# stojicnnnn/3DVision

Hardware: AMD Instinct MI355X
Metric: RANSAC hyps/s + ICP iters/s @ 200k-pt clouds (higher is better)
Workload: dtype f32

## Files before the change

3dvision_amd/__init__.py:

```python
import ctypes as C
import os
import sys
import threading
from dataclasses import dataclass, field
from typing import Optional

import numpy as np

_HERE = os.path.dirname(os.path.abspath(__file__))
STUDY_BUILD = os.environ.get("TDV_LIB_VARIANT") == "study"
LIB_PATH = os.path.join(_HERE, "lib3dvision_hip_study.so" if STUDY_BUILD else "lib3dvision_hip.so")

TDV_MASK_THRESHOLD10 = 0
TDV_MASK_NONZERO = 1
TDV_MASK_LABEL_BASE = 256
TDV_VOXEL_ORDER_FIRST = 0
TDV_VOXEL_ORDER_REFERENCE = 1
TIMER_ICP_NN, TIMER_RANSAC_SCORE, TIMER_FEATURE_MATCH, TIMER_KNN, TIMER_RADIUS, TIMER_DEPTH, TIMER_VOXEL, TIMER_FM_INDEX = range(8)
DEPTH_BATCH_MASK_PASSES = 1

ABI_SYMBOLS = [
    "tdv_device_count", "tdv_ctx_create", "tdv_ctx_set_stream", "tdv_ctx_set_icp_search", "tdv_ctx_set_icp_accumulation", "tdv_ctx_last_icp_search", "tdv_ctx_last_batch_lanes", "tdv_ctx_last_voxel_grouping", "tdv_ctx_last_voxel_batch_redone", "tdv_ctx_last_feature_match_path", "tdv_ctx_workspace_bytes", "tdv_ctx_workspace_fill", "tdv_ctx_set_ransac_score", "tdv_ctx_last_ransac_rescore", "tdv_ctx_last_ransac_scored", "tdv_ctx_last_ransac_bound", "tdv_ctx_get_stream", "tdv_ctx_synchronize",
    "tdv_ctx_destroy", "tdv_status_string", "tdv_last_error", "tdv_version", "tdv_timing_enable", "tdv_timing_read",
    "tdv_depth_preprocess", "tdv_deproject", "tdv_depth_to_cloud", "tdv_voxel_downsample", "tdv_estimate_normals",
    "tdv_compute_fpfh", "tdv_feature_match", "tdv_ransac", "tdv_icp", "tdv_icp_correspondences",
    "tdv_icp_dev", "tdv_ransac_dev", "tdv_feature_match_dev", "tdv_estimate_normals_dev", "tdv_compute_fpfh_dev", "tdv_normals_fpfh_dev", "tdv_radix_sort_pairs_dev",
    "tdv_depth_to_cloud_dev", "tdv_voxel_downsample_dev", "tdv_sample_triples", "tdv_sample_triples_batch", "tdv_pose_compose",
    "tdv_register_batch_dev", "tdv_prepare_model_dev", "tdv_bilateral_filter", "tdv_filter_duplicates", "tdv_ransac_score_unit", "tdv_ransac_score_unit_block", "tdv_ransac_score_unit_chunks", "tdv_ransac_batch_size", "tdv_voxel_rules", "tdv_load_ply_ascii", "tdv_load_mask_png", "tdv_load_masks_from_dir",
    "tdv_depth_to_cloud_batch_dev", "tdv_broadcast_model", "tdv_gather_results", "tdv_mask_resize_nearest", "tdv_mask_resize_nearest_dev", "tdv_voxel_downsample_batch_dev", "tdv_voxel_downsample_batch_pinhole_dev",
    "tdv_icp_batch_dev", "tdv_refine_batch_dev", "tdv_ctx_set_icp_loss", "tdv_ctx_get_icp_loss",
    "tdv_gicp", "tdv_gicp_dev", "tdv_gicp_batch_dev",
    "tdv_color_gradients", "tdv_color_gradients_dev", "tdv_colored_icp", "tdv_colored_icp_dev", "tdv_colored_icp_batch_dev",
    "tdv_fgr_default_params", "tdv_fgr", "tdv_fgr_dev", "tdv_fgr_correspondences",
    "tdv_plane_default_params", "tdv_segment_planes", "tdv_segment_planes_dev",
    "tdv_cluster_default_params", "tdv_cluster_dbscan", "tdv_cluster_dbscan_dev",
    "tdv_remove_statistical_outlier", "tdv_remove_statistical_outlier_dev", "tdv_remove_radius_outlier", "tdv_remove_radius_outlier_dev",
    "tdv_iss_default_params", "tdv_iss_keypoints", "tdv_iss_keypoints_dev",
    "tdv_ppf_default_params", "tdv_ppf_model_bytes", "tdv_ppf_model_dev", "tdv_ppf_match_dev", "tdv_ppf_match",
    "tdv_ppf_match_batch_dev",
    "tdv_farthest_point_down_sample", "tdv_farthest_point_down_sample_dev", "tdv_farthest_point_down_sample_batch_dev",
    "tdv_ctx_set_fps_path", "tdv_ctx_last_fps_path", "tdv_ctx_set_icp_launches", "tdv_ctx_last_icp_launches",
    "tdv_ctx_set_icp_probe_cache", "tdv_ctx_last_icp_probe_misses",
    "tdv_verify_default_params", "tdv_verify_poses", "tdv_verify_poses_dev", "tdv_render_depth", "tdv_render_depth_dev",
    "tdv_mesh_verify_default_params", "tdv_verify_poses_mesh", "tdv_verify_poses_mesh_dev", "tdv_render_depth_mesh", "tdv_render_depth_mesh_dev",
    "tdv_mesh_sample_default_params", "tdv_mesh_sample_points", "tdv_mesh_sample_points_dev",
# ... 507 lines not shown
        _check(self._h, lib().tdv_ctx_set_icp_search(self._h, self.ICP_SEARCH[mode]), "tdv_ctx_set_icp_search")
        self.icp_search_name = mode

    def set_icp_accumulation(self, mode):
        _check(self._h, lib().tdv_ctx_set_icp_accumulation(self._h, {"tree": 0, "reference": 1}[mode]), "tdv_ctx_set_icp_accumulation")

    ICP_LOSS = {"l2": 0, "huber": 1, "tukey": 2, "cauchy": 3}

    def set_icp_loss(self, kind, scale=None):
        if kind not in self.ICP_LOSS:
            raise ValueError("unknown ICP loss %r (one of %s)" % (kind, ", ".join(self.ICP_LOSS)))
        if kind != "l2" and scale is None:
            raise ValueError("the %s loss needs a scale" % kind)
        _check(self._h, lib().tdv_ctx_set_icp_loss(self._h, self.ICP_LOSS[kind], C.c_float(0.0 if scale is None else float(scale))),
               "tdv_ctx_set_icp_loss")

    def icp_loss(self):
        k = C.c_int(); sc = C.c_float()
        _check(self._h, lib().tdv_ctx_get_icp_loss(self._h, C.byref(k), C.byref(sc)), "tdv_ctx_get_icp_loss")
        return {v: n for n, v in self.ICP_LOSS.items()}[k.value], float(sc.value)

    def set_ransac_score(self, mode):
        _check(self._h, lib().tdv_ctx_set_ransac_score(self._h, {"fast": 0, "exact": 1, "matrix": 2}[mode]), "tdv_ctx_set_ransac_score")

    def last_ransac_rescore(self):
        return float(lib().tdv_ctx_last_ransac_rescore(self._h))

    def last_ransac_scored(self):
        return float(lib().tdv_ctx_last_ransac_scored(self._h))

    def last_ransac_bound(self):
        out = (C.c_longlong * 4)()
        lib().tdv_ctx_last_ransac_bound(self._h, out)
        return tuple(int(v) for v in out)

    def last_feature_match_path(self):
        return {0: "none", 1: "scan", 2: "leaf_major", 3: "walk"}[int(lib().tdv_ctx_last_feature_match_path(self._h))]

    def last_voxel_grouping(self):
        return {0: "none", 1: "table", 2: "pixels"}[int(lib().tdv_ctx_last_voxel_grouping(self._h))]

    def last_voxel_batch_redone(self):
        return int(lib().tdv_ctx_last_voxel_batch_redone(self._h))

    def last_batch_lanes(self):
        return int(lib().tdv_ctx_last_batch_lanes(self._h))
# ... 1247 lines not shown
```

3dvision_amd/csrc/batch.hip:

```cpp
#include "tdv_internal.hpp"
#include <algorithm>
#include <functional>
#include <thread>
#include <cstdio>
#include <cstdlib>
#include <cstring>
#include <vector>

namespace tdv {

__global__ void k_globalise(const int* __restrict__ local, const int* __restrict__ voff, int n_inst, int total, int* __restrict__ out) {
    const int P = blockIdx.x * blockDim.x + threadIdx.x;
    if (P >= total) return;
    int a = 0, z = n_inst;
    while (z - a > 1) { const int m = (a + z) >> 1; if (voff[m] <= P) a = m; else z = m; }
    out[P] = local[P] + voff[a];
}

__global__ void k_gather_i32(const int* __restrict__ in, const int* __restrict__ idx, int n, int* __restrict__ out) {
    const int p = blockIdx.x * blockDim.x + threadIdx.x;
    if (p < n) out[p] = in[idx[p]];
}

namespace {
// ... 223 lines not shown
    const bool small_instances = off[n_instances] / std::max(n_instances, 1) < 8192;
    const int lanes_default = std::min(small_instances ? 12 : 3, hw_threads);
    const int want = std::max(1, std::min(std::min(lanes_env > 0 ? lanes_env : lanes_default, 16), n_instances));
    std::vector<tdv_ctx*> lane_ctx{ctx};
    for (tdv_ctx* c = ctx; (int)lane_ctx.size() < want; c = c->helper) {
        if (!c->helper && tdv_ctx_create(ctx->device, &c->helper) != TDV_OK) { c->helper = nullptr; break; }
        lane_ctx.push_back(c->helper);
    }
    const int L = (int)lane_ctx.size();
    ctx->last_batch_lanes = L;
    auto for_all_instances = [&](const std::function<int(tdv_ctx*, int)>& fn) -> int {
        if (L == 1) {
            int st = TDV_OK;
            for (int b = 0; b < n_instances && st == TDV_OK; ++b) st = fn(ctx, b);
            if (hipStreamSynchronize(ctx->stream) != hipSuccess && st == TDV_OK) st = TDV_ERR_LAUNCH;
            return st;
        }
        TDV_HIP(ctx, hipStreamSynchronize(ctx->stream));
        std::vector<int> status((size_t)L, TDV_OK);
        std::vector<std::thread> workers;
        for (int l = 1; l < L; ++l) {
            tdv_ctx* h = lane_ctx[l];
            h->timing = ctx->timing; h->icp_search = ctx->icp_search; h->icp_accumulate = ctx->icp_accumulate;
            h->icp_loss = ctx->icp_loss; h->icp_loss_scale = ctx->icp_loss_scale; h->ransac_score_mode = ctx->ransac_score_mode; h->err[0] = 0;
            workers.emplace_back([&, h, l]() {
                try {
                    if (hipSetDevice(h->device) != hipSuccess) { status[l] = TDV_ERR_NO_DEVICE; return; }
                    status[l] = ws_reset(h);
                    for (int b = l; b < n_instances && status[l] == TDV_OK; b += L) status[l] = fn(h, b);
                    if (hipStreamSynchronize(h->stream) != hipSuccess && status[l] == TDV_OK) status[l] = TDV_ERR_LAUNCH;
                } catch (...) {
                    std::snprintf(h->err, sizeof(h->err), "exception in a helper lane");
                    status[l] = TDV_ERR_INTERNAL;
                }
            });
        }
        try {
            for (int b = 0; b < n_instances && status[0] == TDV_OK; b += L) status[0] = fn(ctx, b);
        } catch (...) {
            std::snprintf(ctx->err, sizeof(ctx->err), "exception in the batch lane");
            status[0] = TDV_ERR_INTERNAL;
        }
        for (auto& w : workers) w.join();
        if (hipStreamSynchronize(ctx->stream) != hipSuccess && status[0] == TDV_OK) status[0] = TDV_ERR_LAUNCH;
        if (status[0] != TDV_OK) return status[0];
        for (int l = 1; l < L; ++l)
            if (status[l] != TDV_OK) { std::snprintf(ctx->err, sizeof(ctx->err), "batch lane %d: %s", l + 1, lane_ctx[l]->err); return status[l]; }
// ... 247 lines not shown
```

3dvision_amd/csrc/ctx.hip:

```cpp
#include "tdv_internal.hpp"
#include <cmath>
#include <cfloat>
#include <algorithm>
#include <cstring>
#include <vector>

namespace tdv {

int ws_reset(tdv_ctx* ctx) {
    if (ctx->blocks.size() > 1) {
        size_t total = 0;
        TDV_HIP(ctx, hipStreamSynchronize(ctx->stream));
        for (auto& b : ctx->blocks) { total += b.cap; (void)hipFree(b.p); }
        ctx->blocks.clear();
        total = align_up(total + total / 4, (size_t)1 << 20);
        char* p = nullptr;
        TDV_HIP(ctx, hipMalloc((void**)&p, total));
        ctx->blocks.push_back({p, total});
    }
    ctx->cur_block = 0; ctx->cur_off = 0; ctx->used_total = 0;
    return TDV_OK;
}

int ws_alloc_bytes(tdv_ctx* ctx, size_t bytes, void** out) {
// ... 274 lines not shown
    if (!ctx || loss < TDV_ICP_LOSS_L2 || loss > TDV_ICP_LOSS_CAUCHY) return TDV_ERR_BAD_ARG;
    if (loss != TDV_ICP_LOSS_L2 && !(std::isfinite(scale) && scale > 0.f)) return TDV_ERR_BAD_ARG;
    ctx->icp_loss = loss;
    ctx->icp_loss_scale = loss == TDV_ICP_LOSS_L2 ? 0.f : scale;
    return TDV_OK;
}

int tdv_ctx_get_icp_loss(tdv_ctx* ctx, int* loss, float* scale) {
    if (!ctx) return TDV_ERR_BAD_ARG;
    if (loss) *loss = ctx->icp_loss;
    if (scale) *scale = ctx->icp_loss_scale;
    return TDV_OK;
}

int tdv_ctx_set_icp_search(tdv_ctx* ctx, int mode) {
    if (!ctx || mode < TDV_ICP_SEARCH_AUTO || mode > TDV_ICP_SEARCH_GRID) return TDV_ERR_BAD_ARG;
    ctx->icp_search = mode;
    return TDV_OK;
}

int tdv_ctx_set_ransac_score(tdv_ctx* ctx, int mode) {
    if (!ctx || (mode != TDV_RANSAC_SCORE_FAST && mode != TDV_RANSAC_SCORE_EXACT && !(tdv::kStudyBuild && mode == TDV_RANSAC_SCORE_MATRIX))) return TDV_ERR_BAD_ARG;
    ctx->ransac_score_mode = mode;
    return TDV_OK;
}

int tdv_ctx_set_fps_path(tdv_ctx* ctx, int mode) {
    if (!ctx || mode < TDV_FPS_AUTO || mode > TDV_FPS_GRID) return TDV_ERR_BAD_ARG;
    ctx->fps_path = mode;
    return TDV_OK;
}
int tdv_ctx_last_fps_path(tdv_ctx* ctx) { return ctx ? ctx->last_fps_path : 0; }

double tdv_ctx_last_ransac_rescore(tdv_ctx* ctx) { return ctx ? ctx->last_ransac_rescore : -1.0; }

double tdv_ctx_last_ransac_scored(tdv_ctx* ctx) { return ctx ? ctx->last_ransac_scored : 1.0; }
void tdv_ctx_last_ransac_bound(tdv_ctx* ctx, long long out[4]) { if (out) for (int e = 0; e < 4; ++e) out[e] = ctx ? ctx->last_ransac_bound[e] : 0; }

int tdv_ctx_last_icp_search(tdv_ctx* ctx) { return ctx ? ctx->last_icp_search : 0; }
int tdv_ctx_last_feature_match_path(tdv_ctx* ctx) { return ctx ? ctx->last_fm_path : 0; }
int tdv_ctx_last_voxel_grouping(tdv_ctx* ctx) { return ctx ? ctx->last_voxel_grouping : 0; }
int tdv_ctx_last_voxel_batch_redone(tdv_ctx* ctx) { return ctx ? ctx->last_voxel_batch_redone : TDV_ERR_BAD_ARG; }
int tdv_ctx_last_batch_lanes(tdv_ctx* ctx) { return ctx ? ctx->last_batch_lanes : 0; }
unsigned long long tdv_ctx_workspace_bytes(tdv_ctx* ctx) {
    unsigned long long total = 0;
    for (tdv_ctx* c = ctx; c; c = c->helper)
// ... 122 lines not shown
```

3dvision_amd/csrc/ransac.hip:

```cpp
#include "tdv_internal.hpp"
#include "host_wait.hpp"
#include "device_linalg.hpp"
#include "ransac_cut.hpp"
#include <cfloat>
#include <climits>
#include <cmath>
#include <cstddef>
#include <cstring>
#include <algorithm>
#include <type_traits>
#include <vector>

namespace tdv {

constexpr float kUnitRoundoff = 5.9604644775390625e-08f;
constexpr float kBandUnit = 16.f * kUnitRoundoff;
constexpr float kBandUnitMatrix = 24.f * kUnitRoundoff;

template <class I>
__device__ __forceinline__ float pair_record(const float* __restrict__ src, const float* __restrict__ tgt, const int* __restrict__ corr, I i, int nt,
                                             int* __restrict__ bad, float4& a, float4& b) {
    int c = corr[i];
    if ((unsigned)c >= (unsigned)nt) { *bad = 1; c = 0; }
    a = make_float4(src[3 * i], src[3 * i + 1], src[3 * i + 2], tgt[3 * c]);
// ... 817 lines not shown
            const int leaf = i / RL_LEAF;
            rl_leaf_store(leaves + (size_t)(leaf >> 1) * 32 + (leaf & 1), min(RL_LEAF, ns - i), bad, lo, hi);
        }
    }
    __syncthreads();
    const int k = threadIdx.x;
    const int i0 = blockIdx.x * 256 + k * RL_COARSE;
    if (k >= 256 / RL_COARSE || i0 >= ns) return;
    float clo[6], chi[6];
    bool cbad = false;
#pragma unroll
    for (int c = 0; c < 6; ++c) { clo[c] = INFINITY; chi[c] = -INFINITY; }
#pragma unroll
    for (int j = 0; j < PER; ++j) {
#pragma unroll
        for (int c = 0; c < 6; ++c) { clo[c] = fminf(clo[c], s_lo[k * PER + j][c]); chi[c] = fmaxf(chi[c], s_hi[k * PER + j][c]); }
        cbad |= s_bad[k * PER + j] != 0;
    }
    const int leaf = i0 / RL_COARSE;
    rl_leaf_store(coarse + (size_t)(leaf >> 1) * 32 + (leaf & 1), min(RL_COARSE, ns - i0), cbad, clo, chi);
}
constexpr int RB_SPLIT = 16;
enum { RB_ONE = 0, RB_COARSE = 1 };
__device__ __forceinline__ int rb_walk(const float* r, const float* __restrict__ leaves, int k0, int k1, float tb, int best, bool done) {
    int ub = 0;
    v2f rr[12], ar[9];
#pragma unroll
    for (int e = 0; e < 12; ++e) rr[e] = (v2f){r[e], r[e]};
#pragma unroll
    for (int e = 0; e < 9; ++e) ar[e] = (v2f){fabsf(r[e]), fabsf(r[e])};
    for (int k = k0; k < k1; ++k) {
        if (((k - k0) & 7) == 0 && !__any(!done)) break;
        const float* __restrict__ g = leaves + (size_t)k * 32;
        float v[32];
#pragma unroll
        for (int e = 0; e < 32; ++e) v[e] = g[e];
        const v2f pcx = {v[0], v[1]}, pcy = {v[2], v[3]}, pcz = {v[4], v[5]};
        const v2f pex = {v[8], v[9]}, pey = {v[10], v[11]}, pez = {v[12], v[13]};
        v2f g2 = {0.f, 0.f};
#pragma unroll
        for (int c = 0; c < 3; ++c) {
            const v2f xc = fma2(rr[c], pcx, fma2(rr[3 + c], pcy, fma2(rr[6 + c], pcz, rr[9 + c])));
            const v2f xe = fma2(ar[c], pex, fma2(ar[3 + c], pey, ar[6 + c] * pez));
            const v2f qlo = {v[16 + 2 * c], v[17 + 2 * c]}, qhi = {v[24 + 2 * c], v[25 + 2 * c]};
            const v2f lo_gap = (xc - xe) - qhi, hi_gap = qlo - (xc + xe);
            const v2f gp = {fmaxf(fmaxf(lo_gap.x, hi_gap.x), 0.f), fmaxf(fmaxf(lo_gap.y, hi_gap.y), 0.f)};
            g2 = fma2(gp, gp, g2);
        }
        const int n2 = (!(g2.x > tb) ? (int)v[6] : 0) + (!(g2.y > tb) ? (int)v[7] : 0);
        if (!done) { ub += n2; done = ub > best; }
    }
    return ub;
}
struct RbHyp { float r[12]; float tb, E; bool bounded; };
__device__ __forceinline__ float rb_band(const float* r, const unsigned* __restrict__ pmax, float sqrt_tau, float band_u) {
    return (band_u * ransac_band_reach(r, __uint_as_float(*pmax)) + band_u * sqrt_tau) * 1.0001f;
// ... 100 lines not shown
    const bool valid = h < count && triples.valid(h);
    const RbHyp o = rb_load(hyp, h_pad, h, valid, pmax, sqrt_tau, band_u, MODE == RB_COARSE ? 5.f : 3.f);
    const int best = state[0];
    const bool walk = rb_gate(best, ns);
    int fl = 0;
    if (wave == 0 && valid) fl = lj.flags[h];
    const int per = (n_lpairs + RB_SPLIT - 1) / RB_SPLIT, k0 = __builtin_amdgcn_readfirstlane(wave) * per, k1 = min(n_lpairs, k0 + per);
    const int ub = rb_walk(o.r, leaves, k0, k1, o.tb, best, !valid || !o.bounded || !walk);
    __syncthreads();
    if (ub) atomicAdd(&s_ub[lane], ub);
    __syncthreads();
    if (wave != 0) return;
    const int total = s_ub[lane];
    const bool gated = valid && (!o.bounded || !walk);
    const bool close = (fl & RB_CLOSE) != 0;
    const bool undecided = MODE == RB_COARSE && valid && !gated && !close && total > best;
    const bool is_live = gated || close || (MODE == RB_ONE && valid && total > best);
    const bool near = is_live && lj.near && (fl & RB_NEAR);
    const unsigned long long mc = __ballot(close);
    if (mc && lane == 0) atomicAdd(lj.n_close, __popcll(mc));
    const int slot = rb_append3(is_live && !near, near, undecided, lane, h, live, n_live, lj.near, lj.n_near, und, n_und);
    if (MODE == RB_COARSE && undecided) acc[slot] = 0;
}
constexpr int RB_FINE_Y = 4;
__global__ __launch_bounds__(64 * RB_SPLIT)
void k_ransac_bound_fine(const float* __restrict__ hyp, int h_pad, const float* __restrict__ leaves, int n_lpairs,
                         const unsigned* __restrict__ pmax, float sqrt_tau, float band_u, const int* __restrict__ state,
                         int* __restrict__ live, int* __restrict__ n_live, const int* __restrict__ und, const int* __restrict__ n_und,
                         int* __restrict__ acc, int* __restrict__ ticket, const ListJob lj) {
    const int lane = threadIdx.x & 63, wave = threadIdx.x >> 6;
    const int n = *n_und, best = state[0];
    const int per_y = (n_lpairs + (int)gridDim.y - 1) / (int)gridDim.y, y0 = blockIdx.y * per_y, y1 = min(n_lpairs, y0 + per_y);
    const int per = (y1 - y0 + RB_SPLIT - 1) / RB_SPLIT;
    const int k0 = min(y1, y0 + __builtin_amdgcn_readfirstlane(wave) * per), k1 = min(y1, k0 + per);
    __shared__ int s_ub[64];
    const int xb = blockIdx.x;
    if (xb * 64 >= n) return;
    const int slot = xb * 64 + lane;
    const int h = slot < n ? und[slot] : -1;
    if (wave == 0) s_ub[lane] = 0;
    const RbHyp o = rb_load(hyp, h_pad, h, h >= 0, pmax, sqrt_tau, band_u, 3.f);
    const int ub = rb_walk(o.r, leaves, k0, k1, o.tb, best, h < 0);
    __syncthreads();
    if (ub) atomicAdd(&s_ub[lane], ub);
    __syncthreads();
    if (wave != 0) return;
    const int part = s_ub[lane];
    if (h >= 0 && part) atomicAdd(&acc[slot], part);
    __threadfence();
    int arrived = 0;
    if (lane == 0) arrived = atomicAdd(&ticket[xb], 1);
    if (__shfl(arrived, 0, 64) != (int)gridDim.y - 1) return;
    const int total = h >= 0 ? atomicAdd(&acc[slot], 0) : 0;
    const bool is_live = h >= 0 && total > best;
    const bool near = is_live && lj.near && (lj.flags[h] & RB_NEAR);
    rb_append3(is_live && !near, near, false, lane, h, live, n_live, lj.near, lj.n_near, nullptr, nullptr);
}

#ifdef TDV_STUDY
#include "ransac_study.hpp"
#endif

__global__ __launch_bounds__(256)
void k_ransac_rmse_partial(const float* __restrict__ pq, int ns, const float* __restrict__ hyp12, float tau,
                           double* __restrict__ slabs) {
    const int i = blockIdx.x * 256 + threadIdx.x;
    double e = 0.0, n = 0.0;
    if (i < ns) {
        const float* g = pq + (size_t)i * 8;
        float px = g[0], py = g[1], pz = g[2];
        float x = (hyp12[0] * px + (hyp12[3] * py + hyp12[6] * pz)) + hyp12[9];
        float y = (hyp12[1] * px + (hyp12[4] * py + hyp12[7] * pz)) + hyp12[10];
        float z = (hyp12[2] * px + (hyp12[5] * py + hyp12[8] * pz)) + hyp12[11];
        float dx = x - g[3], dy = y - g[4], dz = z - g[5];
        float d2 = dx * dx + (dy * dy + dz * dz);
        if (d2 < tau) { float err = sqrtf(d2); e = (double)(err * err); n = 1.0; }
    }
    __shared__ double red[2][4];
#pragma unroll
// ... 46 lines not shown

struct RansacBlock {
    int bad;
    unsigned pmax;
    unsigned long long rescored, scored;
    long long bound[4];
    int state[2];
    int plan[2][8];
    float best12[12];
    double out2[2];
    int sel[4];
    int rec[2][8];
    RansacFar far;
};
constexpr size_t kRansacReadBack = offsetof(RansacBlock, sel);
static_assert(std::is_trivially_copyable<RansacBlock>::value, "memset, copied back");
static_assert(offsetof(RansacBlock, rescored) % 8 == 0 && offsetof(RansacBlock, scored) == offsetof(RansacBlock, rescored) + 8, "the kernels index the two as one u64[2]");
static_assert(offsetof(RansacBlock, out2) % 8 == 0 && offsetof(RansacBlock, out2) + sizeof(double[2]) == kRansacReadBack, "the part read back is a prefix that ends with out2");
struct RansacLive { int n_live[2], n_und[2], n_near[2], n_close[2]; };
static_assert(offsetof(RansacLive, n_und) == offsetof(RansacLive, n_live) + 2 * sizeof(int) && offsetof(RansacLive, n_near) == offsetof(RansacLive, n_live) + 4 * sizeof(int) &&
              offsetof(RansacLive, n_close) == offsetof(RansacLive, n_live) + 6 * sizeof(int), "ransac_plan's n_live[2], n_live[4], n_live[6]");

struct RansacKnobs { bool score_fast, score_mfma, bailout, bound, one_level, leaf_classes, merge, record_copy, upload_inline, order, far, end_event, timer_events; int drop_permille, a_permille, u_cut_permille, fine_y, grown; float far_radius, live_radius; };
static RansacKnobs ransac_knobs(const tdv_ctx* ctx, bool traced, int max_iterations) {
    RansacKnobs k;
    static const bool score_exact_env = getenv("TDV_RANSAC_SCORE") && !strcmp(getenv("TDV_RANSAC_SCORE"), "exact");
    k.score_fast = !score_exact_env && ctx->ransac_score_mode != TDV_RANSAC_SCORE_EXACT;
    const bool score_mfma_env = study_env("TDV_RANSAC_SCORE") && !strcmp(study_env("TDV_RANSAC_SCORE"), "mfma");
    k.score_mfma = kStudyBuild && k.score_fast && (score_mfma_env || ctx->ransac_score_mode == TDV_RANSAC_SCORE_MATRIX);
    static const bool bailout_env_off = getenv("TDV_RANSAC_BAILOUT") && atoi(getenv("TDV_RANSAC_BAILOUT")) == 0;
    k.bailout = k.score_fast && !k.score_mfma && !traced && !bailout_env_off && max_iterations > 16384;
    k.merge = study_env("TDV_RANSAC_MERGE") && atoi(study_env("TDV_RANSAC_MERGE")) == 1;
    const bool bound_env_off = getenv("TDV_RANSAC_BOUND") && atoi(getenv("TDV_RANSAC_BOUND")) == 0;
    k.bound = k.bailout && !k.merge && !bound_env_off;
    const char* const order_env = getenv("TDV_RANSAC_ORDER");
    k.order = k.bailout && !k.merge && !(order_env && atoi(order_env) == 0);
    k.far = k.order && k.bound && !(order_env && atoi(order_env) == 1);
    k.far_radius = study_env("TDV_RANSAC_FAR_RADIUS") ? (float)atof(study_env("TDV_RANSAC_FAR_RADIUS")) : 4.f;
    k.a_permille = study_env("TDV_RANSAC_FAR_A_PERMILLE") ? atoi(study_env("TDV_RANSAC_FAR_A_PERMILLE")) : 110;
    k.u_cut_permille = study_env("TDV_RANSAC_FAR_UCUT_PERMILLE") ? atoi(study_env("TDV_RANSAC_FAR_UCUT_PERMILLE")) : 22;
    k.live_radius = study_env("TDV_RANSAC_LIVE_RADIUS") ? (float)atof(study_env("TDV_RANSAC_LIVE_RADIUS")) : 20.f;
    k.fine_y = study_env("TDV_RANSAC_FINE_Y") ? std::min(std::max(atoi(study_env("TDV_RANSAC_FINE_Y")), 1), 64) : RB_FINE_Y;
    k.grown = study_env("TDV_RANSAC_GROWN") ? (int)align_up((size_t)std::min(std::max(atoi(study_env("TDV_RANSAC_GROWN")), kRansacBatch), 4 * kRansacBatch), RS_HYP_PER_BLOCK) : kRansacGrown;
    k.leaf_classes = study_env("TDV_RANSAC_LEAF_CLASSES") && atoi(study_env("TDV_RANSAC_LEAF_CLASSES")) == 1;
    k.one_level = study_env("TDV_RANSAC_BOUND_LEVELS") && atoi(study_env("TDV_RANSAC_BOUND_LEVELS")) == 1;
    k.record_copy = study_env("TDV_RANSAC_RECORD") && !strcmp(study_env("TDV_RANSAC_RECORD"), "copy");
    k.end_event = traced || k.record_copy || (study_env("TDV_RANSAC_END") && !strcmp(study_env("TDV_RANSAC_END"), "event"));
    k.timer_events = study_env("TDV_RANSAC_TIMER") && !strcmp(study_env("TDV_RANSAC_TIMER"), "events");
    k.upload_inline = study_env("TDV_RANSAC_UPLOAD") && !strcmp(study_env("TDV_RANSAC_UPLOAD"), "inline");
    k.drop_permille = study_env("TDV_RANSAC_DROP_PERMILLE") ? atoi(study_env("TDV_RANSAC_DROP_PERMILLE")) : 50;
    return k;
}

struct RansacBuf {
    float* hyp; int* counts; void* tri; int* list;
    int *live, *und, *acc, *ticket;
    int *near, *list2, *ubf;
    int* flags;
    int* units;
    int *plan, *rec, *n_live, *n_und, *n_near;
    void* h_tri; int* h_cnt; volatile int* h_rec;
    hipEvent_t ev;
    int seq;
};
struct RansacBatch { int q, cnt, it0; bool bounded; };
struct RangeCut { int per, ranges; };
static RangeCut range_cut(int hb, int n_pchunks) {
    const int per = (n_pchunks + point_ranges(hb, n_pchunks) - 1) / point_ranges(hb, n_pchunks);
    return RangeCut{per, (n_pchunks + per - 1) / per};
}
static int hyp_blocks(int cnt) { return (int)(align_up((size_t)cnt, RS_HYP_PER_BLOCK) / RS_HYP_PER_BLOCK); }
static int score_grid(int hb, int ps) { return 8 * ((hb + 8 / RS_XCD_R - 1) / (8 / RS_XCD_R)) * ((ps + RS_XCD_R - 1) / RS_XCD_R); }
static int unit_grid(int cus) { return std::max(8, (2 * cus + 7) / 8 * 8); }

struct RansacRun {
    tdv_ctx* ctx; hipStream_t s; RansacKnobs k;
    int ns, nt, max_iterations; float confidence; int* trace;
    float tau, sqrt_tau, band_u;
    int ns_pad, n_pchunks, batch, cap, h_pad, packed, rblocks, n_lpairs = 0, n_cpairs = 0, cus = 0;
    size_t tri_bytes;
    float *pq = nullptr, *pq2 = nullptr, *pq3 = nullptr, *leaves = nullptr, *cleaves = nullptr; double* slabs = nullptr;
    RansacBlock *d = nullptr, *h = nullptr; RansacLive* lv = nullptr;
    unsigned long long* leaf_keys = nullptr; unsigned* leaf_vals = nullptr; bool leaves_built = false;
    unsigned long long* ord_mask = nullptr; int* ord_cnt = nullptr; bool ordered = false;
    unsigned* enc = nullptr;
    RansacBuf buf[2] = {};
    unsigned long long *stamps = nullptr, *h_stamps = nullptr; int n_stamps = 0, stamps_used = 0;
    RansacBatch pending = {}; bool has_pending = false;
    double wave_chunks = 0.0;
    float best_fitness = 0.f; int best_iter = -1, best_inliers = 0, done_iters = 0; bool stop = false;

    TriView tri(const RansacBuf& B) const { return TriView{B.tri, packed}; }
    int setup(const float* d_src, const float* d_tgt, const int* d_corr) {
        ns_pad = (int)align_up((size_t)ns, (size_t)RS_PCH * 64);
        TDV_TRY(ws_alloc(ctx, (size_t)ns_pad * 8, &pq)); TDV_TRY(ws_alloc(ctx, 1, &d));
        TDV_HIP(ctx, hipMemsetAsync(d, 0, sizeof(RansacBlock), s));
// ... 109 lines not shown
        if (k.score_mfma) wave_chunks += mfma_score(s, B.hyp, h_pad, pq3, ns, b.cnt, tau, B.counts, &d->rescored);
        else
#endif
        if (k.score_fast) {
            const ScoreJob ja{B.hyp, B.counts, nullptr, nullptr, hb, range_cut(hb, n_pchunks).ranges, nullptr, nullptr, nullptr};
            const int gA = score_grid(hb, ja.ps);
            launch_score(gA, ja, ja, gA);
            wave_chunks += (double)hb * (RS_BLOCK / 64) * (double)n_pchunks;
        } else {
            const RangeCut c = range_cut(h_pad / RS_HYP_PER_BLOCK, n_pchunks);
            k_ransac_score<<<dim3(hb, c.ranges), RS_BLOCK, 0, s>>>(B.hyp, h_pad, pq2, n_pchunks, c.per, tau, B.counts);
        }
        return TDV_OK;
    }
    void bound(const RansacBatch& b) {
        const RansacBuf& B = buf[b.q]; const int bgrid = (b.cnt + 63) / 64;
        const ListJob lj{B.flags, k.far ? B.near : nullptr, B.n_near, B.n_live + 6};
        if (k.one_level)
            k_ransac_bound<RB_ONE><<<bgrid, 64 * RB_SPLIT, 0, s>>>(B.hyp, h_pad, tri(B), b.cnt, leaves, n_lpairs, &d->pmax, sqrt_tau, band_u,
                                                                   d->state, ns, B.live, B.n_live, nullptr, nullptr, nullptr, nullptr, lj);
        else {
            k_ransac_bound<RB_COARSE><<<bgrid, 64 * RB_SPLIT, 0, s>>>(B.hyp, h_pad, tri(B), b.cnt, cleaves, n_cpairs, &d->pmax, sqrt_tau, band_u,
                                                                      d->state, ns, B.live, B.n_live, B.und, B.n_und, B.acc, B.ticket, lj);
            k_ransac_bound_fine<<<dim3(bgrid, k.fine_y), 64 * RB_SPLIT, 0, s>>>(B.hyp, h_pad, leaves, n_lpairs, &d->pmax, sqrt_tau, band_u,
                                                                                  d->state, B.live, B.n_live, B.und, B.n_und, B.acc, B.ticket, lj);
        }
    }
    void point_order() {
        RansacFar* const far = k.far ? &d->far : nullptr;
        k_order_flags<<<order_blocks(), RO_BLOCK, 0, s>>>(pq, ns, d->state, d->best12, tau, ord_mask, ord_cnt, far, std::max(tau, k.far_radius * k.far_radius * tau));
        k_order_scatter<<<order_blocks(), RO_BLOCK, 0, s>>>(pq, ns, ord_mask, ord_cnt, pq2, far);
        ordered = true;
    }
    ScoreJob job_a(const RansacBatch& b) const { return ScoreJob{buf[b.q].hyp, buf[b.q].counts, buf[b.q].plan, nullptr, hyp_blocks(b.cnt), range_cut(hyp_blocks(b.cnt), n_pchunks).ranges, nullptr, nullptr, nullptr}; }
    void phase1(const RansacBatch& b) {
        const RansacBuf& B = buf[b.q];
        const int hbw = slots(b.cnt) / RS_BLOCK;
        const ScoreJob ja = job_a(b), jl{B.hyp, B.counts, B.plan, B.live, hbw, 0, B.n_live, B.units, nullptr};
        const ScoreJob jn = k.far ? ScoreJob{B.hyp, B.counts, B.plan, B.near, hbw, 0, B.n_near, B.units + 16 * hbw, &d->far.c_far} : jl;
        const int g1 = score_grid(ja.hb, ja.ps);
        ScopedTimer tm(ctx, score_slot());
        if (b.bounded) launch_score(unit_grid(cus), jn, jl, 0);
        else launch_score(g1, ja, ja, g1);
    }
    int select(const RansacBatch& b) {
        const RansacBuf& B = buf[b.q];
        if (b.bounded) k_ransac_select_live<<<1, 1024, 0, s>>>(B.live, B.n_live, k.far ? B.near : nullptr, B.n_near, B.ubf, B.counts, ns, confidence, d->state, B.plan, B.list, B.list2);
        else {
// ... 146 lines not shown
        pose_to_T16(h->best12, out->T);
        out->fitness = best_fitness; out->inliers = best_inliers; out->best_iteration = best_iter;
        out->rmse = best_inliers > 0 ? std::sqrt((float)h->out2[0] / (float)best_inliers) : 999.0f;
        if ((int)(h->out2[1] + 0.5) != best_inliers) {
            snprintf(ctx->err, sizeof(ctx->err), "ransac: rmse pass counted %d inliers, scoring pass %d", (int)(h->out2[1] + 0.5), best_inliers);
            return TDV_ERR_INTERNAL;
        }
        return TDV_OK;
    }
};

int ransac_run_dev(tdv_ctx* ctx, const float* d_src, int ns, const float* d_tgt, int nt, const float* d_fs, const float* d_ft, const int* d_corr_in,
                   float voxel, int max_iterations, float confidence, uint32_t seed, tdv_ransac_result* out, int* trace_inliers) {
    if (!ctx || !out || ns < 0 || nt < 0 || max_iterations < 0) return TDV_ERR_BAD_ARG;
    if (ns > 0 && (!d_src || !d_tgt)) return TDV_ERR_BAD_ARG;
    if (!d_corr_in && ns > 0 && nt > 0 && (!d_fs || !d_ft)) return TDV_ERR_BAD_ARG;
    TDV_HIP(ctx, hipSetDevice(ctx->device));
    result_defaults(out);
    if (ns == 0 || nt == 0 || max_iterations == 0) return TDV_OK;
    int* d_match = nullptr;
    if (!d_corr_in) { TDV_TRY(ws_alloc(ctx, (size_t)ns, &d_match)); TDV_TRY(feature_match_dev(ctx, d_fs, ns, d_ft, nt, d_match)); }
    const int* d_corr = d_corr_in ? d_corr_in : d_match;
    RansacRun r;
    r.ctx = ctx; r.s = ctx->stream; r.k = ransac_knobs(ctx, trace_inliers != nullptr, max_iterations);
    r.ns = ns; r.nt = nt; r.max_iterations = max_iterations; r.confidence = confidence; r.trace = trace_inliers;
    r.tau = tau_lt(voxel * 1.5f);
    r.sqrt_tau = std::nextafter((float)std::sqrt((double)r.tau), INFINITY);
    r.band_u = r.k.score_mfma ? kBandUnitMatrix : kBandUnit;
    TDV_TRY(r.setup(d_src, d_tgt, d_corr));
    const int status = r.loop(seed);
    (void)hipStreamSynchronize(r.s);
    ctx->last_ransac_rescore = -1.0; ctx->last_ransac_scored = 1.0;
    for (long long& v : ctx->last_ransac_bound) v = 0;
    r.release_events();
    return status != TDV_OK ? status : r.result(out);
}


struct RbResult { float T[12]; int best_iter, inliers, iterations_run, pad; };

__global__ __launch_bounds__(1024)
void k_rb_sample(const unsigned* __restrict__ raw, int n_raw, const int* __restrict__ off, int H, int* __restrict__ idx_out , int* __restrict__ fail) {
    const int b = blockIdx.x, n = off[b + 1] - off[b];
    if (n <= 0) return;
    const unsigned range = (unsigned)n, thr = (0u - range) % range;
    int* out = idx_out + (size_t)b * 3 * H;
    __shared__ int s_wave[16];
// ... 196 lines not shown
```

3dvision_amd/csrc/ransac_cut.hpp:

```cpp
#pragma once
#include <hip/hip_runtime.h>

#ifndef RS_WG_TARGET
#define RS_WG_TARGET 6144
#endif
#ifndef RS_UNIT
#define RS_UNIT 16
#endif

namespace tdv {

__host__ __device__ __forceinline__ int point_ranges(int hb, int n_pchunks) { return min(min((RS_WG_TARGET + hb - 1) / hb, max(1, n_pchunks / 32)), 512); }

__host__ __device__ __forceinline__ bool score_unit(int ticket, int r0, int r1, int xcd, int& c0, int& c1) {
    const int n = r1 > r0 ? r1 - r0 : 0, share = (n + 7) / 8;
    const int x0 = min(n, xcd * share), x1 = min(n, x0 + share);
    if (ticket < 0 || ticket > share / RS_UNIT) return false;
    c0 = r0 + x0 + ticket * RS_UNIT; c1 = min(r0 + x1, c0 + RS_UNIT);
    return c0 < c1;
}
__host__ __device__ __forceinline__ int score_unit_block(int wg, int visit, int n_blk) { return (int)(((unsigned)wg + (unsigned)visit) % (unsigned)n_blk); }

constexpr int kRansacFirst = 8192, kRansacBatch = 65536, kRansacGrown = 131072;
constexpr int kRansacGrowAt = kRansacFirst + 4 * kRansacBatch;
__host__ __device__ __forceinline__ int ransac_batch_size(int it0, int grown = kRansacGrown) {
    return it0 == 0 ? kRansacFirst : it0 < kRansacGrowAt ? kRansacBatch : grown;
}

}
```

3dvision_amd/csrc/tdv_internal.hpp:

```cpp
#pragma once
#include <hip/hip_runtime.h>
#include <climits>
#include <cmath>
#include <cstdint>
#include <cstdio>
#include <cstdlib>
#include <cstring>
#include <vector>
#include "tdv_hip.h"
#include "depth_frames.hpp"

namespace tdv {

struct TimerSlot {
    double total_ms = 0.0;
    int launches = 0;
    std::vector<std::pair<hipEvent_t, hipEvent_t>> pending;
};

}

struct tdv_ctx {
    int device = 0;
    hipStream_t stream = nullptr;
    bool own_stream = false;
    struct Block { char* p; size_t cap; };
    std::vector<Block> blocks;
    size_t cur_block = 0, cur_off = 0, high_water = 0, used_total = 0;
    char* pin = nullptr;
    size_t pin_cap = 0;
    char err[512] = {0};
    bool timing = false;
    int icp_search = 0;
    int icp_accumulate = 0;
    int icp_loss = 0;
    float icp_loss_scale = 0.f;
    int ransac_score_mode = 0;
    double last_ransac_rescore = -1.0;
    long long last_ransac_bound[4] = {0, 0, 0, 0};
    double last_ransac_scored = 1.0;
    int last_voxel_grouping = 0;
    int last_voxel_batch_redone = -1;
    int last_fm_path = 0;
    int last_batch_lanes = 0;
    int fps_path = 0;
    int last_fps_path = 0;
    int icp_launches = 0;
    int last_icp_launches = 0;
    int icp_probe_cache = 0;
    int last_icp_probe_misses = -1;
    int last_icp_search = 0;
    unsigned* scan_ticket = nullptr;
    unsigned long long* chain_status = nullptr;
    size_t chain_cap = 0;
    unsigned chain_epoch = 0, chain_ticket_base = 0;
    tdv_ctx* helper = nullptr;
    tdv::TimerSlot timers[TDV_TIMER_COUNT];
    std::vector<hipEvent_t> event_pool;
    int ransac_seq = 0;
// ... 239 lines not shown
```

include/tdv_hip.h:

```cpp
#ifndef TDV_HIP_H
#define TDV_HIP_H

#include <stddef.h>
#include <stdint.h>

#ifdef __cplusplus
extern "C" {
#endif

typedef struct tdv_ctx tdv_ctx;

typedef enum tdv_status {
    TDV_OK = 0,
    TDV_ERR_NO_DEVICE = -1,
    TDV_ERR_BAD_ARG = -2,
    TDV_ERR_OOM = -3,
    TDV_ERR_LAUNCH = -4,
    TDV_ERR_INTERNAL = -5
} tdv_status;

int tdv_device_count(int* count);
int tdv_ctx_create(int device, tdv_ctx** out);
int tdv_ctx_set_stream(tdv_ctx* ctx, void* hip_stream);
void* tdv_ctx_get_stream(tdv_ctx* ctx);
// ... 7 lines not shown
#define TDV_ICP_ACCUMULATE_TREE 0
#define TDV_ICP_ACCUMULATE_REFERENCE 1
int tdv_ctx_set_icp_accumulation(tdv_ctx* ctx, int mode);
#define TDV_ICP_LAUNCHES_AUTO 0
#define TDV_ICP_LAUNCHES_TWO 1
#define TDV_ICP_LAUNCHES_ONE 2
int tdv_ctx_set_icp_launches(tdv_ctx* ctx, int mode);
int tdv_ctx_last_icp_launches(tdv_ctx* ctx);
#define TDV_ICP_PROBE_CACHE_AUTO 0
#define TDV_ICP_PROBE_CACHE_OFF 1
#define TDV_ICP_PROBE_CACHE_ON 2
int tdv_ctx_set_icp_probe_cache(tdv_ctx* ctx, int mode);
int tdv_ctx_last_icp_probe_misses(tdv_ctx* ctx);
#define TDV_ICP_LOSS_L2 0
#define TDV_ICP_LOSS_HUBER 1
#define TDV_ICP_LOSS_TUKEY 2
#define TDV_ICP_LOSS_CAUCHY 3
int tdv_ctx_set_icp_loss(tdv_ctx* ctx, int loss, float scale);
int tdv_ctx_get_icp_loss(tdv_ctx* ctx, int* loss, float* scale);
#define TDV_RANSAC_SCORE_FAST 0
#define TDV_RANSAC_SCORE_EXACT 1
#define TDV_RANSAC_SCORE_MATRIX 2
int tdv_ctx_set_ransac_score(tdv_ctx* ctx, int mode);
double tdv_ctx_last_ransac_rescore(tdv_ctx* ctx);
double tdv_ctx_last_ransac_scored(tdv_ctx* ctx);
int tdv_ctx_last_icp_search(tdv_ctx* ctx);
#define TDV_FM_PATH_SCAN 1
#define TDV_FM_PATH_LEAF_MAJOR 2
#define TDV_FM_PATH_WALK 3
int tdv_ctx_last_feature_match_path(tdv_ctx* ctx);
#define TDV_VOXEL_GROUPING_TABLE 1
#define TDV_VOXEL_GROUPING_PIXELS 2
int tdv_ctx_last_voxel_grouping(tdv_ctx* ctx);
int tdv_ctx_last_voxel_batch_redone(tdv_ctx* ctx);
int tdv_ctx_last_batch_lanes(tdv_ctx* ctx);
unsigned long long tdv_ctx_workspace_bytes(tdv_ctx* ctx);
int tdv_ctx_workspace_fill(tdv_ctx* ctx, int byte);
const char* tdv_status_string(int status);
const char* tdv_last_error(tdv_ctx* ctx);
const char* tdv_version(void);

#define TDV_TIMER_ICP_NN 0
#define TDV_TIMER_RANSAC_SCORE 1
#define TDV_TIMER_FEATURE_MATCH 2
#define TDV_TIMER_KNN 3
#define TDV_TIMER_RADIUS 4
// ... 546 lines not shown
```

Measured before the change: 8739.

## Make RANSAC fine bound kernel persistent with adaptive range split and leaf-class auto

The fine bound kernel becomes a persistent grid-stride loop sized to the CU count. Inside the kernel it picks the number of leaf ranges from a cost model (rounds times walk length plus overhead), replacing the fixed 4-way y split. Leaves and job parameters are read through the constant (kernarg) address space so they can use scalar loads. Leaf-class ordering is also enabled automatically for clouds with at least 50k correspondences, and a new API knob selects the leaf order. This aims to balance work across CUs and cut register pressure, with the risk that a poor cost-model choice or the leaf-class switch lowers throughput.

```diff
diff --git a/3dvision_amd/__init__.py b/3dvision_amd/__init__.py
--- a/3dvision_amd/__init__.py
+++ b/3dvision_amd/__init__.py
@@ -20,7 +20,7 @@
 DEPTH_BATCH_MASK_PASSES = 1
 
 ABI_SYMBOLS = [
-    "tdv_device_count", "tdv_ctx_create", "tdv_ctx_set_stream", "tdv_ctx_set_icp_search", "tdv_ctx_set_icp_accumulation", "tdv_ctx_last_icp_search", "tdv_ctx_last_batch_lanes", "tdv_ctx_last_voxel_grouping", "tdv_ctx_last_voxel_batch_redone", "tdv_ctx_last_feature_match_path", "tdv_ctx_workspace_bytes", "tdv_ctx_workspace_fill", "tdv_ctx_set_ransac_score", "tdv_ctx_last_ransac_rescore", "tdv_ctx_last_ransac_scored", "tdv_ctx_last_ransac_bound", "tdv_ctx_get_stream", "tdv_ctx_synchronize",
+    "tdv_device_count", "tdv_ctx_create", "tdv_ctx_set_stream", "tdv_ctx_set_icp_search", "tdv_ctx_set_icp_accumulation", "tdv_ctx_last_icp_search", "tdv_ctx_last_batch_lanes", "tdv_ctx_last_voxel_grouping", "tdv_ctx_last_voxel_batch_redone", "tdv_ctx_last_feature_match_path", "tdv_ctx_workspace_bytes", "tdv_ctx_workspace_fill", "tdv_ctx_set_ransac_score", "tdv_ctx_set_ransac_leaf_order", "tdv_ctx_last_ransac_rescore", "tdv_ctx_last_ransac_scored", "tdv_ctx_last_ransac_bound", "tdv_ctx_get_stream", "tdv_ctx_synchronize",
     "tdv_ctx_destroy", "tdv_status_string", "tdv_last_error", "tdv_version", "tdv_timing_enable", "tdv_timing_read",
     "tdv_depth_preprocess", "tdv_deproject", "tdv_depth_to_cloud", "tdv_voxel_downsample", "tdv_estimate_normals",
     "tdv_compute_fpfh", "tdv_feature_match", "tdv_ransac", "tdv_icp", "tdv_icp_correspondences",
@@ -574,6 +574,9 @@
 
     def set_ransac_score(self, mode):
         _check(self._h, lib().tdv_ctx_set_ransac_score(self._h, {"fast": 0, "exact": 1, "matrix": 2}[mode]), "tdv_ctx_set_ransac_score")
+
+    def set_ransac_leaf_order(self, mode):
+        _check(self._h, lib().tdv_ctx_set_ransac_leaf_order(self._h, {"auto": 0, "morton": 1, "classes": 2}[mode]), "tdv_ctx_set_ransac_leaf_order")
 
     def last_ransac_rescore(self):
         return float(lib().tdv_ctx_last_ransac_rescore(self._h))
diff --git a/3dvision_amd/csrc/batch.hip b/3dvision_amd/csrc/batch.hip
--- a/3dvision_amd/csrc/batch.hip
+++ b/3dvision_amd/csrc/batch.hip
@@ -269,7 +269,7 @@
         for (int l = 1; l < L; ++l) {
             tdv_ctx* h = lane_ctx[l];
             h->timing = ctx->timing; h->icp_search = ctx->icp_search; h->icp_accumulate = ctx->icp_accumulate;
-            h->icp_loss = ctx->icp_loss; h->icp_loss_scale = ctx->icp_loss_scale; h->ransac_score_mode = ctx->ransac_score_mode; h->err[0] = 0;
+            h->icp_loss = ctx->icp_loss; h->icp_loss_scale = ctx->icp_loss_scale; h->ransac_score_mode = ctx->ransac_score_mode; h->ransac_leaf_order = ctx->ransac_leaf_order; h->err[0] = 0;
             workers.emplace_back([&, h, l]() {
                 try {
                     if (hipSetDevice(h->device) != hipSuccess) { status[l] = TDV_ERR_NO_DEVICE; return; }
diff --git a/3dvision_amd/csrc/ctx.hip b/3dvision_amd/csrc/ctx.hip
--- a/3dvision_amd/csrc/ctx.hip
+++ b/3dvision_amd/csrc/ctx.hip
@@ -320,6 +320,12 @@
 int tdv_ctx_set_ransac_score(tdv_ctx* ctx, int mode) {
     if (!ctx || (mode != TDV_RANSAC_SCORE_FAST && mode != TDV_RANSAC_SCORE_EXACT && !(tdv::kStudyBuild && mode == TDV_RANSAC_SCORE_MATRIX))) return TDV_ERR_BAD_ARG;
     ctx->ransac_score_mode = mode;
+    return TDV_OK;
+}
+
+int tdv_ctx_set_ransac_leaf_order(tdv_ctx* ctx, int mode) {
+    if (!ctx || mode < TDV_RANSAC_LEAVES_AUTO || mode > TDV_RANSAC_LEAVES_CLASSES) return TDV_ERR_BAD_ARG;
+    ctx->ransac_leaf_order = mode;
     return TDV_OK;
 }
 
diff --git a/3dvision_amd/csrc/ransac.hip b/3dvision_amd/csrc/ransac.hip
--- a/3dvision_amd/csrc/ransac.hip
+++ b/3dvision_amd/csrc/ransac.hip
@@ -863,7 +863,9 @@
 }
 constexpr int RB_SPLIT = 16;
 enum { RB_ONE = 0, RB_COARSE = 1 };
-__device__ __forceinline__ int rb_walk(const float* r, const float* __restrict__ leaves, int k0, int k1, float tb, int best, bool done) {
+typedef const float __attribute__((address_space(4)))* RbConstLeaves;
+template <typename LeafPtr>
+__device__ __forceinline__ int rb_walk(const float* r, const LeafPtr leaves, int k0, int k1, float tb, int best, bool done) {
     int ub = 0;
     v2f rr[12], ar[9];
 #pragma unroll
@@ -872,7 +874,7 @@
     for (int e = 0; e < 9; ++e) ar[e] = (v2f){fabsf(r[e]), fabsf(r[e])};
     for (int k = k0; k < k1; ++k) {
         if (((k - k0) & 7) == 0 && !__any(!done)) break;
-        const float* __restrict__ g = leaves + (size_t)k * 32;
+        const LeafPtr g = leaves + (size_t)k * 32;
         float v[32];
 #pragma unroll
         for (int e = 0; e < 32; ++e) v[e] = g[e];
@@ -1019,39 +1021,62 @@
     const int slot = rb_append3(is_live && !near, near, undecided, lane, h, live, n_live, lj.near, lj.n_near, und, n_und);
     if (MODE == RB_COARSE && undecided) acc[slot] = 0;
 }
-constexpr int RB_FINE_Y = 4;
+struct FineJob {
+    const float* hyp; const float* leaves; const unsigned* pmax; const int* state; const int* und; const int* n_und;
+    int *live, *n_live, *acc, *ticket; ListJob lj;
+    int h_pad, n_lpairs, force_y; float sqrt_tau, band_u;
+};
+typedef const FineJob __attribute__((address_space(4)))* FineJobArg;
 __global__ __launch_bounds__(64 * RB_SPLIT)
-void k_ransac_bound_fine(const float* __restrict__ hyp, int h_pad, const float* __restrict__ leaves, int n_lpairs,
-                         const unsigned* __restrict__ pmax, float sqrt_tau, float band_u, const int* __restrict__ state,
-                         int* __restrict__ live, int* __restrict__ n_live, const int* __restrict__ und, const int* __restrict__ n_und,
-                         int* __restrict__ acc, int* __restrict__ ticket, const ListJob lj) {
-    const int lane = threadIdx.x & 63, wave = threadIdx.x >> 6;
-    const int n = *n_und, best = state[0];
-    const int per_y = (n_lpairs + (int)gridDim.y - 1) / (int)gridDim.y, y0 = blockIdx.y * per_y, y1 = min(n_lpairs, y0 + per_y);
-    const int per = (y1 - y0 + RB_SPLIT - 1) / RB_SPLIT;
-    const int k0 = min(y1, y0 + __builtin_amdgcn_readfirstlane(wave) * per), k1 = min(y1, k0 + per);
+void k_ransac_bound_fine(const FineJob job) {
+    const int lane = threadIdx.x & 63, wave = __builtin_amdgcn_readfirstlane(threadIdx.x >> 6);
+    const int n = *job.n_und, best = job.state[0], n_lpairs = job.n_lpairs;
+    const int nb = (n + 63) / 64;
+    int ranges = job.force_y > 0 ? job.force_y : 1;
+    if (job.force_y <= 0 && nb > 0) {
+        unsigned long long key = fine_cut_key(lane + 1, nb, n_lpairs, (int)gridDim.x, RB_SPLIT);
+#pragma unroll
+        for (int off = 32; off > 0; off >>= 1) { const unsigned long long o = __shfl_xor(key, off, 64); key = o < key ? o : key; }
+        ranges = __builtin_amdgcn_readfirstlane((int)(key & 127ull));
+    }
+    const int per_y = (n_lpairs + ranges - 1) / ranges, units = nb * ranges;
+    const RbConstLeaves leaves = (RbConstLeaves)job.leaves;
     __shared__ int s_ub[64];
-    const int xb = blockIdx.x;
-    if (xb * 64 >= n) return;
-    const int slot = xb * 64 + lane;
-    const int h = slot < n ? und[slot] : -1;
-    if (wave == 0) s_ub[lane] = 0;
-    const RbHyp o = rb_load(hyp, h_pad, h, h >= 0, pmax, sqrt_tau, band_u, 3.f);
-    const int ub = rb_walk(o.r, leaves, k0, k1, o.tb, best, h < 0);
-    __syncthreads();
-    if (ub) atomicAdd(&s_ub[lane], ub);
-    __syncthreads();
-    if (wave != 0) return;
-    const int part = s_ub[lane];
-    if (h >= 0 && part) atomicAdd(&acc[slot], part);
-    __threadfence();
-    int arrived = 0;
-    if (lane == 0) arrived = atomicAdd(&ticket[xb], 1);
-    if (__shfl(arrived, 0, 64) != (int)gridDim.y - 1) return;
-    const int total = h >= 0 ? atomicAdd(&acc[slot], 0) : 0;
-    const bool is_live = h >= 0 && total > best;
-    const bool near = is_live && lj.near && (lj.flags[h] & RB_NEAR);
-    rb_append3(is_live && !near, near, false, lane, h, live, n_live, lj.near, lj.n_near, nullptr, nullptr);
+#pragma unroll 1
+    for (int u = blockIdx.x; u < units; u += (int)gridDim.x) {
+        FineJobArg j = (FineJobArg)__builtin_amdgcn_kernarg_segment_ptr();
+        asm volatile("" : "+s"(j));
+        const int y = u / nb, xb = u - y * nb;
+        const int y0 = min(n_lpairs, y * per_y), y1 = min(n_lpairs, y0 + per_y);
+        const int per = (y1 - y0 + RB_SPLIT - 1) / RB_SPLIT;
+        const int k0 = min(y1, y0 + wave * per), k1 = min(y1, k0 + per);
+        const int slot = xb * 64 + lane;
+        const int h = slot < n ? j->und[slot] : -1;
+        if (wave == 0) s_ub[lane] = 0;
+        const RbHyp o = rb_load(j->hyp, j->h_pad, h, h >= 0, j->pmax, j->sqrt_tau, j->band_u, 3.f);
+        const int ub = rb_walk(o.r, leaves, k0, k1, o.tb, best, h < 0);
+        __syncthreads();
+        if (ub) atomicAdd(&s_ub[lane], ub);
+        __syncthreads();
+        if (wave != 0) continue;
+        int tl = lane;
+        asm volatile("" : "+v"(tl));
+        FineJobArg t = (FineJobArg)__builtin_amdgcn_kernarg_segment_ptr();
+        asm volatile("" : "+s"(t));
+        const int tslot = xb * 64 + tl;
+        const int part = s_ub[tl];
+        int* const acc = t->acc;
+        if (h >= 0 && part) atomicAdd(&acc[tslot], part);
+        __threadfence();
+        int arrived = 0;
+        if (tl == 0) arrived = atomicAdd(&t->ticket[xb], 1);
+        if (__shfl(arrived, 0, 64) != ranges - 1) continue;
+        const int total = h >= 0 ? atomicAdd(&acc[tslot], 0) : 0;
+        const bool is_live = h >= 0 && total > best;
+        int* const nearl = t->lj.near;
+        const bool near = is_live && nearl && (t->lj.flags[h] & RB_NEAR);
+        rb_append3(is_live && !near, near, false, tl, h, t->live, t->n_live, nearl, t->lj.n_near, nullptr, nullptr);
+    }
 }
 
 #ifdef TDV_STUDY
@@ -1144,7 +1169,7 @@
               offsetof(RansacLive, n_close) == offsetof(RansacLive, n_live) + 6 * sizeof(int), "ransac_plan's n_live[2], n_live[4], n_live[6]");
 
 struct RansacKnobs { bool score_fast, score_mfma, bailout, bound, one_level, leaf_classes, merge, record_copy, upload_inline, order, far, end_event, timer_events; int drop_permille, a_permille, u_cut_permille, fine_y, grown; float far_radius, live_radius; };
-static RansacKnobs ransac_knobs(const tdv_ctx* ctx, bool traced, int max_iterations) {
+static RansacKnobs ransac_knobs(const tdv_ctx* ctx, bool traced, int max_iterations, int ns) {
     RansacKnobs k;
     static const bool score_exact_env = getenv("TDV_RANSAC_SCORE") && !strcmp(getenv("TDV_RANSAC_SCORE"), "exact");
     k.score_fast = !score_exact_env && ctx->ransac_score_mode != TDV_RANSAC_SCORE_EXACT;
@@ -1162,9 +1187,10 @@
     k.a_permille = study_env("TDV_RANSAC_FAR_A_PERMILLE") ? atoi(study_env("TDV_RANSAC_FAR_A_PERMILLE")) : 110;
     k.u_cut_permille = study_env("TDV_RANSAC_FAR_UCUT_PERMILLE") ? atoi(study_env("TDV_RANSAC_FAR_UCUT_PERMILLE")) : 22;
     k.live_radius = study_env("TDV_RANSAC_LIVE_RADIUS") ? (float)atof(study_env("TDV_RANSAC_LIVE_RADIUS")) : 20.f;
-    k.fine_y = study_env("TDV_RANSAC_FINE_Y") ? std::min(std::max(atoi(study_env("TDV_RANSAC_FINE_Y")), 1), 64) : RB_FINE_Y;
+    k.fine_y = study_env("TDV_RANSAC_FINE_Y") ? std::min(std::max(atoi(study_env("TDV_RANSAC_FINE_Y")), 1), kFineMaxRanges) : 0;
     k.grown = study_env("TDV_RANSAC_GROWN") ? (int)align_up((size_t)std::min(std::max(atoi(study_env("TDV_RANSAC_GROWN")), kRansacBatch), 4 * kRansacBatch), RS_HYP_PER_BLOCK) : kRansacGrown;
-    k.leaf_classes = study_env("TDV_RANSAC_LEAF_CLASSES") && atoi(study_env("TDV_RANSAC_LEAF_CLASSES")) == 1;
+    k.leaf_classes = ctx->ransac_leaf_order == TDV_RANSAC_LEAVES_CLASSES || (ctx->ransac_leaf_order == TDV_RANSAC_LEAVES_AUTO && ns >= kRansacLeafClassesMin);
+    if (study_env("TDV_RANSAC_LEAF_CLASSES")) k.leaf_classes = atoi(study_env("TDV_RANSAC_LEAF_CLASSES")) == 1;
     k.one_level = study_env("TDV_RANSAC_BOUND_LEVELS") && atoi(study_env("TDV_RANSAC_BOUND_LEVELS")) == 1;
     k.record_copy = study_env("TDV_RANSAC_RECORD") && !strcmp(study_env("TDV_RANSAC_RECORD"), "copy");
     k.end_event = traced || k.record_copy || (study_env("TDV_RANSAC_END") && !strcmp(study_env("TDV_RANSAC_END"), "event"));
@@ -1194,6 +1220,7 @@
 static int hyp_blocks(int cnt) { return (int)(align_up((size_t)cnt, RS_HYP_PER_BLOCK) / RS_HYP_PER_BLOCK); }
 static int score_grid(int hb, int ps) { return 8 * ((hb + 8 / RS_XCD_R - 1) / (8 / RS_XCD_R)) * ((ps + RS_XCD_R - 1) / RS_XCD_R); }
 static int unit_grid(int cus) { return std::max(8, (2 * cus + 7) / 8 * 8); }
+static int fine_grid(int cus) { return unit_grid(cus); }
 
 struct RansacRun {
     tdv_ctx* ctx; hipStream_t s; RansacKnobs k;
@@ -1349,8 +1376,8 @@
         else {
             k_ransac_bound<RB_COARSE><<<bgrid, 64 * RB_SPLIT, 0, s>>>(B.hyp, h_pad, tri(B), b.cnt, cleaves, n_cpairs, &d->pmax, sqrt_tau, band_u,
                                                                       d->state, ns, B.live, B.n_live, B.und, B.n_und, B.acc, B.ticket, lj);
-            k_ransac_bound_fine<<<dim3(bgrid, k.fine_y), 64 * RB_SPLIT, 0, s>>>(B.hyp, h_pad, leaves, n_lpairs, &d->pmax, sqrt_tau, band_u,
-                                                                                  d->state, B.live, B.n_live, B.und, B.n_und, B.acc, B.ticket, lj);
+            const FineJob fj{B.hyp, leaves, &d->pmax, d->state, B.und, B.n_und, B.live, B.n_live, B.acc, B.ticket, lj, h_pad, n_lpairs, k.fine_y, sqrt_tau, band_u};
+            k_ransac_bound_fine<<<fine_grid(cus), 64 * RB_SPLIT, 0, s>>>(fj);
         }
     }
     void point_order() {
@@ -1543,7 +1570,7 @@
     if (!d_corr_in) { TDV_TRY(ws_alloc(ctx, (size_t)ns, &d_match)); TDV_TRY(feature_match_dev(ctx, d_fs, ns, d_ft, nt, d_match)); }
     const int* d_corr = d_corr_in ? d_corr_in : d_match;
     RansacRun r;
-    r.ctx = ctx; r.s = ctx->stream; r.k = ransac_knobs(ctx, trace_inliers != nullptr, max_iterations);
+    r.ctx = ctx; r.s = ctx->stream; r.k = ransac_knobs(ctx, trace_inliers != nullptr, max_iterations, ns);
     r.ns = ns; r.nt = nt; r.max_iterations = max_iterations; r.confidence = confidence; r.trace = trace_inliers;
     r.tau = tau_lt(voxel * 1.5f);
     r.sqrt_tau = std::nextafter((float)std::sqrt((double)r.tau), INFINITY);
diff --git a/3dvision_amd/csrc/ransac_cut.hpp b/3dvision_amd/csrc/ransac_cut.hpp
--- a/3dvision_amd/csrc/ransac_cut.hpp
+++ b/3dvision_amd/csrc/ransac_cut.hpp
@@ -27,4 +27,22 @@
     return it0 == 0 ? kRansacFirst : it0 < kRansacGrowAt ? kRansacBatch : grown;
 }
 
+constexpr int kRansacLeafClassesMin = 50000;
+static_assert(kRansacLeafClassesMin > 30000, "the suite compares Morton lists at 30,000 pairs");
+
+constexpr int kFineUnitCost = 6, kFineMinWalk = 8, kFineMaxRanges = 64;
+__host__ __device__ __forceinline__ unsigned long long fine_cut_key(int r, int nb, int n_lpairs, int grid, int waves) {
+    if (r < 1 || r > kFineMaxRanges) return ~0ull;
+    const int walk = ((n_lpairs + r - 1) / r + waves - 1) / waves;
+    if (r > 1 && walk < kFineMinWalk) return ~0ull;
+    const unsigned units = (unsigned)nb * (unsigned)r, rounds = (units + (unsigned)grid - 1u) / (unsigned)grid;
+    return ((unsigned long long)rounds * (unsigned)(walk + kFineUnitCost)) << 7 | (unsigned)r;
 }
+__host__ __device__ __forceinline__ int fine_ranges(int nb, int n_lpairs, int grid, int waves) {
+    if (nb <= 0 || grid <= 0) return 1;
+    unsigned long long best = ~0ull;
+    for (int r = 1; r <= kFineMaxRanges; ++r) { const unsigned long long k = fine_cut_key(r, nb, n_lpairs, grid, waves); best = k < best ? k : best; }
+    return (int)(best & 127ull);
+}
+
+}
diff --git a/3dvision_amd/csrc/tdv_internal.hpp b/3dvision_amd/csrc/tdv_internal.hpp
--- a/3dvision_amd/csrc/tdv_internal.hpp
+++ b/3dvision_amd/csrc/tdv_internal.hpp
@@ -35,6 +35,7 @@
     int icp_accumulate = 0;
     int icp_loss = 0;
     float icp_loss_scale = 0.f;
+    int ransac_leaf_order = 0;
     int ransac_score_mode = 0;
     double last_ransac_rescore = -1.0;
     long long last_ransac_bound[4] = {0, 0, 0, 0};
diff --git a/include/tdv_hip.h b/include/tdv_hip.h
--- a/include/tdv_hip.h
+++ b/include/tdv_hip.h
@@ -53,6 +53,10 @@
 #define TDV_RANSAC_SCORE_EXACT 1
 #define TDV_RANSAC_SCORE_MATRIX 2
 int tdv_ctx_set_ransac_score(tdv_ctx* ctx, int mode);
+#define TDV_RANSAC_LEAVES_AUTO 0
+#define TDV_RANSAC_LEAVES_MORTON 1
+#define TDV_RANSAC_LEAVES_CLASSES 2
+int tdv_ctx_set_ransac_leaf_order(tdv_ctx* ctx, int mode);
 double tdv_ctx_last_ransac_rescore(tdv_ctx* ctx);
 double tdv_ctx_last_ransac_scored(tdv_ctx* ctx);
 int tdv_ctx_last_icp_search(tdv_ctx* ctx);
```

After: 9464, median of 6. 8.3% higher.
